# marzer/rt

Measured on AMD Instinct MI355X. Metric: Mrays/s (W*H*spp per second) and wall-clock, 1920x1080x256spp scenes/basic.toml, higher is better.
Workload: dtype f32

## Files before the change

rt_amd/csrc/kernels.hip:

```cpp
#include "kernels.hpp"
#include "contract.hpp"
#include "scan.hpp"
#include "bvh_scan.hpp"

#ifdef RT_HIP_FAST_BUILD
#define render_queue render_queue_fast
#define launch_render launch_render_fast
#endif

#include "../../include/rt_hip.h"

#include <algorithm>
#include <cstdlib>

#ifndef RT_HIP_WAVES_FEW
#define RT_HIP_WAVES_FEW 7
#endif
#ifndef RT_HIP_WAVES_MANY
#define RT_HIP_WAVES_MANY 6
#endif
#ifndef RT_HIP_WAVES_RESIDENT
#define RT_HIP_WAVES_RESIDENT 7
#endif
#ifndef RT_HIP_WAVES_DENSE
// ... 214 lines not shown
		}

		__device__ __forceinline__ uint32_t count_arrival(uint32_t* counter)
		{
#ifdef RT_HIP_MODEL_ORDERING
			return __hip_atomic_fetch_add(counter, 1u, __ATOMIC_RELEASE, __HIP_MEMORY_SCOPE_AGENT);
#else
			asm volatile("s_waitcnt vmcnt(0) ; what was published has left before the arrival is counted" ::: "memory");
			return __hip_atomic_fetch_add(counter, 1u, __ATOMIC_RELAXED, __HIP_MEMORY_SCOPE_AGENT);
#endif
		}
		__device__ __forceinline__ void last_arrival()
		{
#ifdef RT_HIP_MODEL_ORDERING
			__builtin_amdgcn_fence(__ATOMIC_ACQUIRE, "agent");
#else
			__builtin_amdgcn_fence(__ATOMIC_ACQUIRE, "wavefront");
#endif
		}

		template <int NS, bool SM, bool HALF = false, int NP = 0, bool GC = false>
		__global__ __launch_bounds__(block_threads, NS == -4 ? RT_HIP_WAVES_BVH : NS == -3 ? RT_HIP_WAVES_DENSE : (NS < 0 ? 5 : (NS == 0 ? RT_HIP_WAVES_RESIDENT : (NS >= 6 && NS + NP >= 7 ? RT_HIP_WAVES_MANY : RT_HIP_WAVES_FEW)))) void render_queue(const frame_params p,
																	  const queue_params q,
																	  const small_scene small,
																	  const device_scene s,
																	  const float4* __restrict__ geometry,
																	  uint32_t* __restrict__ out_rgba,
																	  float* __restrict__ out_rgb,
																	  device_counters* __restrict__ counters,
																	  unsigned long long* item_sums,
																	  uint32_t* pixel_done)
		{
			extern __shared__ float4 lds[];
			float4* const lds_geometry = lds;
			float4* const lds_shading = lds + scalar_max_spheres;
			constexpr bool RESIDENT = NS == 0;
			constexpr bool RESIDENT_SCALAR_SCAN = NS == 0 && NP == 1;
			const bool spheres_in_lds = RESIDENT && !RESIDENT_SCALAR_SCAN;
			const uint32_t lds_spheres = spheres_in_lds ? s.n_spheres : 0u;
			constexpr bool BVH = NS == -4;
			const uint32_t table_float4s = NS > 0 ? small_table_float4s : (RESIDENT ? lds_spheres + s.n_planes : (NS == -1 ? tile_primitives : (BVH ? bvh_stack_float4s : 0u)));
			if (NS > 0)
			{
				if (threadIdx.x == 0)
				{
#pragma unroll
					for (int i = 0; i < NS + NP; i++)
					{
						lds_geometry[i] = make_float4(small.geometry[i].x, small.geometry[i].y, small.geometry[i].z, __uint_as_float(small.scatter[i]));
						lds_shading[i] = small.shading[i];
					}
				}
			}
			else if (RESIDENT)
			{
				for (uint32_t i = threadIdx.x; i < lds_spheres + s.n_planes; i += block_threads)
					lds[i] = s.primitive_geometry[(s.n_spheres - lds_spheres) + i];
			}
			__syncthreads();

#ifdef RT_HIP_REGION_COUNTERS
			uint32_t region_runs[device_counters::regions] = {}, region_lanes[device_counters::regions] = {};
#endif
			constexpr bool ROLLING = NS < 0 && !BVH;
			device_bvh bvh{};
			if constexpr (BVH)
				bvh = *reinterpret_cast<const device_bvh*>(item_sums);
			constexpr bool RESIDENT_LDS_SCAN = NS == 0 && NP == 0;
			constexpr bool PINHOLE_ONLY = (NS > 0 || RESIDENT_LDS_SCAN) && !GC, EYE_ONLY = NS > 0 && GC, NEVER_PINHOLE = RESIDENT_LDS_SCAN && GC;
			const uint32_t lane = threadIdx.x & 63u;
			const uint32_t wave = threadIdx.x >> 6;
			const uint32_t chunk_items = q.chunks << q.pixels_log2;
			const uint32_t items = HALF ? 2u * chunk_items : chunk_items;
			constexpr uint32_t slot_floats = HALF ? half_chunk_slot_floats : 3u;
			float* const slots = reinterpret_cast<float*>(lds + table_float4s) + static_cast<size_t>(wave) * chunk_items * slot_floats;
			const uint32_t tile_w = 1u << q.tile_w_log2;
			const uint32_t tile_h = (1u << q.pixels_log2) >> q.tile_w_log2;

			const uint32_t tile_x0 = (blockIdx.x * 4u + wave) * tile_w;
			const uint32_t tile_y0 = (gridDim.y - 1u - blockIdx.y) * tile_h;
			uint32_t next_item = 0;

			const uint32_t items_per_pixel = (ROLLING && HALF) ? (p.samples_per_pixel + q.item_samples - 1u) / q.item_samples : q.chunks;
			const unsigned long long total_items = static_cast<unsigned long long>(p.width) * p.local_rows * items_per_pixel;
			unsigned long long block_next = 0, block_end = 0;
			unsigned long long prefetched = 0;
			uint32_t prefetched_count = ROLLING ? min(64u, q.lane_cap) : 64u;
			bool dry = false;
			if (ROLLING)
				prefetched = fetch_items(counters, prefetched_count);
#ifdef RT_HIP_WAVE_CLOCKS
			const unsigned long long clock_start = wall_clock64();
			unsigned long long clock_dry = 0;
#endif

			lane_state st;
			constexpr bool SCALAR_SEGMENTS = NS >= 1 && NS + NP <= 4;
			unsigned long long wave_segments = 0;
			uint32_t lane_segments = 0;
			uint32_t slot = 0;
			enum : uint32_t { lane_free = 0, lane_restart = 1, lane_retired = 3, lane_trace = 4 };
			uint32_t mode = lane_free;
#define RT_HIP_IS(m) ((m) == lane_trace ? mode >= lane_trace : mode == (m))
#define RT_HIP_BECOME(m) (mode = (m))

			const auto fold_tile = [&](const float* sums, uint32_t x0, uint32_t y0)
			{
				if (!ROLLING && (3u << q.pixels_log2) <= 64u)
				{
					const uint32_t channel = lane >> q.pixels_log2;
					const uint32_t pixel = lane & ((1u << q.pixels_log2) - 1u);
					const uint32_t lx = x0 + (pixel & (tile_w - 1u));
					const uint32_t ly = y0 + (pixel >> q.tile_w_log2);
					const bool live = channel < 3u && lx < p.width && ly < p.local_rows;
					float sum = 0.0f;
					if (live)
					{
						if (HALF)
						{
							for (uint32_t c = 0; c < q.chunks; c++)
							{
								const float* const slot_of_chunk = sums + ((c << q.pixels_log2) + pixel) * slot_floats;
								float chunk_sum = slot_of_chunk[channel];
								const uint32_t parked = parked_samples(p.samples_per_pixel, c);
								for (uint32_t j = 0; j < parked; j++)
									chunk_sum = chunk_sum + slot_of_chunk[3u + j * 3u + channel];
								sum = c ? sum + chunk_sum : chunk_sum;
							}
						}
						else
						{
							sum = sums[pixel * 3u + channel];
							for (uint32_t c = 1; c < q.chunks; c++)
								sum = sum + sums[((c << q.pixels_log2) + pixel) * 3u + channel];
						}
					}
					const float mean = sum / static_cast<float>(p.samples_per_pixel);
					const size_t o = static_cast<size_t>(output_row(live ? ly : 0u, p)) * p.width + lx;
					if (live && out_rgb)
						out_rgb[o * 3u + channel] = mean;
					const uint32_t byte = static_cast<uint32_t>(clamp01(__builtin_sqrtf(mean)) * 255.99999f);
					const uint32_t green = __shfl(byte, lane + (1u << q.pixels_log2), 64);
					const uint32_t blue = __shfl(byte, lane + (2u << q.pixels_log2), 64);
					if (live && channel == 0u)
						__hip_atomic_store(&out_rgba[o], (byte << 24u) | (green << 16u) | (blue << 8u) | 255u, __ATOMIC_RELAXED, __HIP_MEMORY_SCOPE_SYSTEM);
					return;
				}
				for (uint32_t pixel = lane; pixel < (1u << q.pixels_log2); pixel += 64u)
				{
					const uint32_t lx = x0 + (pixel & (tile_w - 1u));
					const uint32_t ly = y0 + (pixel >> q.tile_w_log2);
					if (lx < p.width && ly < p.local_rows)
					{
						vec3 colour = { 0.0f, 0.0f, 0.0f };
						if (HALF)
						{
							for (uint32_t c = 0; c < q.chunks; c++)
							{
								const float* const slot_of_chunk = sums + ((c << q.pixels_log2) + pixel) * slot_floats;
								vec3 chunk_sum = { slot_of_chunk[0], slot_of_chunk[1], slot_of_chunk[2] };
								const uint32_t parked = parked_samples(p.samples_per_pixel, c);
								for (uint32_t j = 0; j < parked; j++)
									chunk_sum = chunk_sum + vec3{ slot_of_chunk[3u + j * 3u], slot_of_chunk[4u + j * 3u], slot_of_chunk[5u + j * 3u] };
								colour = c ? colour + chunk_sum : chunk_sum;
							}
						}
						else
						{
							colour = { sums[pixel * 3u], sums[pixel * 3u + 1u], sums[pixel * 3u + 2u] };
							for (uint32_t c = 1; c < q.chunks; c++)
							{
								const uint32_t at = ((c << q.pixels_log2) + pixel) * 3u;
								colour = colour + vec3{ sums[at], sums[at + 1u], sums[at + 2u] };
							}
						}
						finish_pixel(colour, p, lx, ly, out_rgba, out_rgb);
					}
				}
			};
			const auto complete_item = [&]()
			{
				const uint32_t row = slot / p.width;
				const uint32_t lx = slot - row * p.width;
				const uint32_t ly = p.local_rows - 1u - row;
				if (HALF)
				{
					unsigned long long* const samples = item_sums + 2u * static_cast<size_t>(slot) * p.samples_per_pixel;
					const uint32_t before = count_arrival(&pixel_done[slot]);
					if (before + 1u == items_per_pixel)
					{
						last_arrival();
						vec3 colour = { 0.0f, 0.0f, 0.0f };
						for (uint32_t first = 0; first < p.samples_per_pixel; first += sample_chunk)
						{
							const uint32_t end = min(first + sample_chunk, p.samples_per_pixel);
							vec3 chunk_sum = { 0.0f, 0.0f, 0.0f };
							uint32_t i = first;
							for (; i + 8u <= end; i += 8u)
							{
								vec3 value[8];
								read_sums8(samples + 2u * i, value);
#pragma unroll
								for (uint32_t k = 0; k < 8u; k++)
									chunk_sum = chunk_sum + value[k];
							}
							for (; i < end; i++)
								chunk_sum = chunk_sum + read_sum(samples + 2u * i);
							colour = first ? colour + chunk_sum : chunk_sum;
						}
						finish_pixel(colour, p, lx, ly, out_rgba, out_rgb);
					}
					return;
				}
				if (q.chunks == 1u)
				{
					finish_pixel(st.chunk_sum, p, lx, ly, out_rgba, out_rgb);
					return;
				}
				const uint32_t chunk = (st.sample_end - 1u) / sample_chunk;
				unsigned long long* const sums = item_sums + 2u * static_cast<size_t>(slot) * q.chunks;
				publish_sum(sums + 2u * chunk, st.chunk_sum);
				const uint32_t before = count_arrival(&pixel_done[slot]);
				if (before + 1u == q.chunks)
				{
					last_arrival();
					vec3 colour = read_sum(sums);
					for (uint32_t c = 1; c < q.chunks; c++)
						colour = colour + read_sum(sums + 2u * c);
					finish_pixel(colour, p, lx, ly, out_rgba, out_rgb);
				}
			};

			constexpr bool INDEXED = HALF || ROLLING;
			const auto next_sample = [&]() -> bool
			{
#ifdef RT_HIP_FAST_BUILD
				st.window += st.keys.stride << draws_per_sample_log2;
#else
				asm("v_lshl_add_u32 %0, %1, %2, %0" : "+v"(st.window) : "v"(st.keys.stride), "n"(draws_per_sample_log2));
#endif
				if (INDEXED)
					return ++st.sample < st.sample_end;
				return st.window != st.window_end;
			};

			const auto end_sample = [&](vec3 contribution)
			{
				if (HALF && ROLLING)
				{
					publish_sum(item_sums + 2u * (static_cast<size_t>(slot) * p.samples_per_pixel + st.sample), contribution);
					if (next_sample())
						RT_HIP_BECOME(lane_restart);
					else
					{
						complete_item();
						RT_HIP_BECOME(lane_free);
					}
					return;
				}
				if (HALF)
				{
					const uint32_t half_chunk = slot >> q.pixels_log2;
					float* const slot_of_chunk = slots + ((((half_chunk >> 1u) << q.pixels_log2) + (slot & ((1u << q.pixels_log2) - 1u))) * slot_floats);
					if (st.sample & 8u)
					{
						float* const place = slot_of_chunk + 3u + (st.sample & 7u) * 3u;
						place[0] = contribution.x;
						place[1] = contribution.y;
						place[2] = contribution.z;
					}
					else
						st.chunk_sum = st.chunk_sum + contribution;
					if (next_sample())
						RT_HIP_BECOME(lane_restart);
					else
					{
						if (!((st.sample - 1u) & 8u))
						{
							slot_of_chunk[0] = st.chunk_sum.x;
							slot_of_chunk[1] = st.chunk_sum.y;
							slot_of_chunk[2] = st.chunk_sum.z;
						}
						RT_HIP_BECOME(lane_free);
					}
					return;
				}
				st.chunk_sum = st.chunk_sum + contribution;
				if (next_sample())
					RT_HIP_BECOME(lane_restart);
				else
				{
					if (ROLLING)
						complete_item();
					else
					{
						slots[slot * 3u + 0u] = st.chunk_sum.x;
						slots[slot * 3u + 1u] = st.chunk_sum.y;
						slots[slot * 3u + 2u] = st.chunk_sum.z;
					}
					RT_HIP_BECOME(lane_free);
				}
			};

			while (true)
			{
				RT_HIP_REGION(0);
				const bool tracing = RT_HIP_IS(lane_trace);
				if (SCALAR_SEGMENTS)
					wave_segments += static_cast<unsigned>(__builtin_popcountll(__builtin_amdgcn_ballot_w64(tracing)));
				candidate tiled_planes = { 0.0f, 0u, false };
				candidate tiled_spheres = { 0.0f, 0u, false };
				if (NS == -1 && __syncthreads_or(tracing))
				{
					for (uint32_t first = 0; first < s.n_planes; first += tile_primitives)
					{
						const uint32_t count = min(tile_primitives, s.n_planes - first);
						__syncthreads();
						stage_planes(lds, s, first, count);
						__syncthreads();
						if (tracing)
							scan_lds<false>(tiled_planes, st.origin, st.dir, lds, count, first);
					}
					for (uint32_t first = 0; first < s.n_spheres; first += tile_primitives)
					{
						const uint32_t count = min(tile_primitives, s.n_spheres - first);
						__syncthreads();
						stage_spheres(lds, s, first, count);
						__syncthreads();
						if (tracing)
							scan_lds<true>(tiled_spheres, st.origin, st.dir, lds, count, first);
					}
				}

				candidate together = { 0.0f, 0u, false };
				bool scanned_together = false;
#ifdef RT_HIP_NO_SPARSE_WAVES
				constexpr bool sparse_waves = false;
#else
				constexpr bool sparse_waves = true;
#endif
				if (sparse_waves && NS == -2 && s.n_spheres >= sparse_min_spheres)
				{
					unsigned long long holders = __builtin_amdgcn_ballot_w64(tracing);
					if (holders != 0 && static_cast<uint32_t>(__builtin_popcountll(holders)) <= q.sparse_rays)
					{
						while (holders != 0)
						{
							const int src = __builtin_ctzll(holders);
							holders &= holders - 1u;
							const vec3 o = { __int_as_float(__builtin_amdgcn_readlane(__float_as_int(st.origin.x), src)), __int_as_float(__builtin_amdgcn_readlane(__float_as_int(st.origin.y), src)),
											 __int_as_float(__builtin_amdgcn_readlane(__float_as_int(st.origin.z), src)) };
							const vec3 d = { __int_as_float(__builtin_amdgcn_readlane(__float_as_int(st.dir.x), src)), __int_as_float(__builtin_amdgcn_readlane(__float_as_int(st.dir.y), src)),
											 __int_as_float(__builtin_amdgcn_readlane(__float_as_int(st.dir.z), src)) };
							candidate found;
							const bool clean = scan_spheres_together(found, o, d, geometry, s.n_spheres, lane);
							if (clean && lane == static_cast<uint32_t>(src))
							{
								together = found;
								scanned_together = true;
							}
						}
					}
				}

				bool shade = false;
				vec3 normal;
				float4 shading;
				uint32_t scatter_kind = scatter_lambert;
				if (tracing)
				{
					RT_HIP_REGION(1);
					if (!SCALAR_SEGMENTS)
						lane_segments++;
					uint32_t kind;
					float distance;
					uint32_t small_index = 0;
					if (NS == -1)
					{
						uint32_t index;
						kind = select_hit(tiled_spheres, tiled_planes, distance, index);
						fetch_hit<SM>(s, st.origin, st.dir, kind, distance, index, normal, shading, scatter_kind);
					}
					else if (NS > 0)
					{
						candidate best = { 0.0f, 0u, false };
						constexpr int spheres_ns = NS > 0 ? NS : 1;
#ifdef RT_HIP_PROBE_GROUP
						constexpr int group = RT_HIP_PROBE_GROUP;
#else
						constexpr int group = spheres_ns <= 4 ? spheres_ns : 3;
#endif
#pragma unroll
						for (int first = 0; first < NS; first += group)
						{
							sphere_probe probes[group];
							unsigned long long lanes[group];
							unsigned long long any_lane = 0;
#pragma unroll
							for (int i = 0; i < group; i++)
								if (first + i < NS)
								{
									probes[i] = probe_sphere(st.origin, st.dir, small.geometry[first + i]);
									lanes[i] = __builtin_amdgcn_ballot_w64(probes[i].pos);
									any_lane |= lanes[i];
								}
							if (any_lane != 0)
							{
#pragma unroll
								for (int i = 0; i < group; i++)
									if (first + i < NS)
									{
										if (lanes[i] != 0)
											RT_HIP_REGION(2);
										finish_sphere(best, probes[i], small.geometry[first + i].w, static_cast<uint32_t>(first + i), lanes[i]);
									}
							}
						}
						if (NP > 0)
						{
							float plane_distance;
							uint32_t plane_slot = static_cast<uint32_t>(NS);
							bool plane;
							if (NP == 1)
								plane = test_one_plane(st.origin, st.dir, small.geometry[NS > 0 ? NS : 0], plane_distance);
							else
							{
								candidate best_plane = { 0.0f, 0u, false };
#pragma unroll
								for (int j = 0; j < NP; j++)
									test_plane(best_plane, st.origin, st.dir, small.geometry[(NS > 0 ? NS : 0) + j], static_cast<uint32_t>(j));
								plane = best_plane.have && best_plane.t >= 0.0f;
								plane_distance = best_plane.t;
								plane_slot += best_plane.index;
							}
							const bool nearer = best.t <= plane_distance;
							const bool sphere = best.have && best.t >= 0.0f;
							const bool use_sphere = sphere && (!plane || nearer);
							const bool use_plane = plane && !use_sphere;
							distance = use_sphere ? best.t : plane_distance;
							kind = use_sphere ? 1u : (use_plane ? 2u : 0u);
							small_index = use_sphere ? best.index : plane_slot;
						}
						else
						{
							const bool hit = best.have && best.t >= 0.0f;
							kind = hit ? 1u : 0u;
							distance = best.t;
							small_index = best.index;
						}
					}
					else
					{
						candidate planes = { 0.0f, 0u, false };
						candidate spheres = { 0.0f, 0u, false };
						const float4* const primitives = RESIDENT ? lds : geometry;
						scan_lds<false>(planes, st.origin, st.dir, RESIDENT ? lds + lds_spheres : geometry + s.n_spheres, s.n_planes, 0);
						if (BVH)
						{
							if (!bvh_spheres(spheres, st.origin, st.dir, bvh, geometry, reinterpret_cast<uint32_t*>(lds) + threadIdx.x))
							{
								spheres = { 0.0f, 0u, false };
								scan_streamed_spheres(spheres, st.origin, st.dir, geometry, s.n_spheres);
							}
#ifdef RT_HIP_BVH_CHECK
							candidate linear = { 0.0f, 0u, false };
							scan_streamed_spheres(linear, st.origin, st.dir, geometry, s.n_spheres);
							const bool same = linear.have == spheres.have && (!linear.have || (__float_as_uint(linear.t) == __float_as_uint(spheres.t) && linear.index == spheres.index));
							atomicAdd(&counters->bvh_checked, 1ull);
							if (!same)
								atomicAdd(&counters->bvh_disagreements, 1ull);
#endif
						}
						else if (NS == -2 || NS == -3)
						{
							if (scanned_together)
								spheres = together;
							else
								scan_streamed_spheres(spheres, st.origin, st.dir, geometry, s.n_spheres);
						}
						else if (RESIDENT_SCALAR_SCAN)
							scan_streamed_spheres(spheres, st.origin, st.dir, geometry, s.n_spheres);
						else
							scan_lds<true>(spheres, st.origin, st.dir, primitives, s.n_spheres, 0);
						uint32_t index;
						kind = select_hit(spheres, planes, distance, index);
						fetch_hit<SM>(s, st.origin, st.dir, kind, distance, index, normal, shading, scatter_kind);
					}
					if (!kind)
					{
						RT_HIP_REGION(4);
						end_sample(st.throughput * sky(st.dir.y));
					}
					else
					{
						shade = true;
						st.origin = ray_at(st.origin, st.dir, distance);
						if (NS > 0)
						{
							RT_HIP_REGION(3);
							const float4 g = lds_geometry[small_index];
							shading = lds_shading[small_index];
							scatter_kind = __float_as_uint(g.w);
							if (NP > 0 && kind == 2u)
								normal = { g.x, g.y, g.z };
							else
							{
								if (NP > 0)
									asm volatile("; hit: some lane hit a sphere" ::: "memory");
								normal = normalize(st.origin - vec3{ g.x, g.y, g.z });
							}
						}
					}
				}


				const unsigned long long asking = __builtin_amdgcn_ballot_w64(RT_HIP_IS(lane_free));
				const auto start_item = [&](uint32_t lx, uint32_t ly, uint32_t chunk)
				{
					const uint32_t item_samples = (HALF && ROLLING) ? q.item_samples : (HALF ? sample_chunk / 2u : sample_chunk);
					if (HALF && !ROLLING && chunk * item_samples >= p.samples_per_pixel)
						return;
					const uint32_t gy = global_row(ly, p);
					st.chunk_sum = { 0.0f, 0.0f, 0.0f };
					{
						const float fx = static_cast<float>(lx), fy = static_cast<float>(gy);
						if (PINHOLE_ONLY || (!EYE_ONLY && !NEVER_PINHOLE && p.pinhole))
						{
							st.base_x = fma(p.ray_d1[0], fx, fma(p.ray_d2[0], fy, p.ray_d0[0]));
							st.base_y = fma(p.ray_d1[1], fx, fma(p.ray_d2[1], fy, p.ray_d0[1]));
							st.base_z = fma(p.ray_d1[2], fx, fma(p.ray_d2[2], fy, p.ray_d0[2]));
							st.base_w = 0.0f;
						}
						else if (EYE_ONLY || p.eye_form)
						{
							st.base_x = fma(p.eye_q1[0], fx, fma(p.eye_q2[0], fy, p.eye_q0[0]));
							st.base_y = fma(p.eye_q1[1], fx, fma(p.eye_q2[1], fy, p.eye_q0[1]));
							st.base_z = fma(p.eye_q1[2], fx, fma(p.eye_q2[2], fy, p.eye_q0[2]));
							st.base_w = fma(p.eye_w1, fx, fma(p.eye_w2, fy, p.eye_w0));
						}
						else
						{
							st.base_x = fx, st.base_y = fy;
							st.base_z = st.base_w = 0.0f;
						}
					}
					st.keys.function_key = pixel_function_key(p.frame_key_a, gy * p.width + lx);
					st.keys.stride = pixel_stride(p.frame_key_b, st.keys.function_key);
					const uint32_t first = chunk * item_samples, end = min(first + item_samples, p.samples_per_pixel);
					st.sample = first;
					st.sample_end = end;
					st.window = sample_counter(st.keys.stride, first);
					st.window_end = sample_counter(st.keys.stride, end);
					RT_HIP_BECOME(lane_restart);
				};
				const auto take_item = [&](uint32_t item, uint32_t x0, uint32_t y0)
				{
					const uint32_t pixel = item & ((1u << q.pixels_log2) - 1u);
					const uint32_t chunk = item >> q.pixels_log2;
					const uint32_t lx = x0 + (pixel & (tile_w - 1u));
					const uint32_t ly = y0 + (pixel >> q.tile_w_log2);
					if (lx < p.width && ly < p.local_rows)
						start_item(lx, ly, chunk);
				};
				if (!ROLLING && asking != 0)
				{
					RT_HIP_REGION(6);
					const uint32_t rank = __builtin_amdgcn_mbcnt_hi(static_cast<uint32_t>(asking >> 32), __builtin_amdgcn_mbcnt_lo(static_cast<uint32_t>(asking), 0u));
					if (RT_HIP_IS(lane_free))
					{
						slot = next_item + rank;
						if (slot >= items)
							RT_HIP_BECOME(lane_retired);
						else
						{
							RT_HIP_REGION(7);
							take_item(slot, tile_x0, tile_y0);
						}
					}
					next_item += static_cast<uint32_t>(__builtin_popcountll(asking));
				}
				if (ROLLING && asking != 0)
				{
					const uint32_t rank = __builtin_amdgcn_mbcnt_hi(static_cast<uint32_t>(asking >> 32), __builtin_amdgcn_mbcnt_lo(static_cast<uint32_t>(asking), 0u));
					uint32_t want = static_cast<uint32_t>(__builtin_popcountll(asking));
					if (q.lane_cap < 64u)
					{
						const uint32_t holding = static_cast<uint32_t>(__builtin_popcountll(__builtin_amdgcn_ballot_w64(RT_HIP_IS(lane_trace) || RT_HIP_IS(lane_restart))));
						want = min(want, q.lane_cap > holding ? q.lane_cap - holding : 0u);
					}
					uint32_t served = 0;
					while (served < want)
					{
						if (block_next == block_end)
						{
							if (dry)
								break;
							if (prefetched >= total_items)
							{
								dry = true;
#ifdef RT_HIP_WAVE_CLOCKS
								clock_dry = wall_clock64();
#endif
								break;
							}
							block_next = prefetched;
							block_end = min(prefetched + prefetched_count, total_items);
// ... 687 lines not shown
```

rt_amd/csrc/scan.hpp:

```cpp
#pragma once

#include "contract.hpp"
#include "kernels.hpp"

namespace rt_hip
{
	constexpr uint32_t block_threads = 256;

	struct candidate
	{
		float t;
		uint32_t index;
		bool have;
	};

	struct sphere_probe
	{
		float a, e2, disc;
		bool pos;
	};

	__device__ __forceinline__ sphere_probe probe_sphere(vec3 o, vec3 d, float4 s)
	{
		const vec3 e = { s.x - o.x, s.y - o.y, s.z - o.z };
		sphere_probe p;
		p.a = dot(e, d);
		p.e2 = dot(e, e);
		p.disc = s.w - fma(-p.a, p.a, p.e2);
		p.pos = !(p.disc < 0.0f);
		return p;
	}

	__device__ __forceinline__ void finish_sphere(candidate& best, const sphere_probe& p, float r2, uint32_t index, unsigned long long lanes)
	{
		if (lanes != 0)
		{
			const float f = sqrt_rn_where(p.disc, p.pos);
			const float t = (p.e2 < r2) ? p.a + f : p.a - f;
			const bool accept = p.pos && !(t < min_hit_dist) && !(best.have && best.t <= t);
			best.t = accept ? t : best.t;
			best.index = accept ? index : best.index;
			best.have = best.have || accept;
		}
	}

	__device__ __forceinline__ void test_sphere(candidate& best, vec3 o, vec3 d, float4 s, uint32_t index)
	{
		const sphere_probe p = probe_sphere(o, d, s);
		finish_sphere(best, p, s.w, index, __builtin_amdgcn_ballot_w64(p.pos));
	}

	__device__ __forceinline__ void test_plane(candidate& best, vec3 o, vec3 d, float4 pl, uint32_t index)
	{
		const vec3 n = { pl.x, pl.y, pl.z };
		const float den = dot(n, d);
		const bool crosses = !(__builtin_fabsf(den) <= approx_zero_epsilon);
		const float num = dot(n, o) + pl.w;
		const float t = (-num) * rcp_rn_not_tiny_where(den, crosses);
		const bool accept = crosses && !(t < min_hit_dist) && !(best.have && best.t <= t);
		best.t = accept ? t : best.t;
		best.index = accept ? index : best.index;
		best.have = best.have || accept;
	}

	__device__ __forceinline__ bool test_one_plane(vec3 o, vec3 d, float4 pl, float& t)
	{
		const vec3 n = { pl.x, pl.y, pl.z };
		const float den = dot(n, d);
		const bool crosses = !(__builtin_fabsf(den) <= approx_zero_epsilon);
		const float num = dot(n, o) + pl.w;
		t = (-num) * rcp_in_band(den);
		return crosses && t >= min_hit_dist;
	}

	template <bool SPHERES>
	__device__ __forceinline__ void scan_lds(candidate& best, vec3 o, vec3 d, const float4* lds, uint32_t count, uint32_t first_index)
	{
		uint32_t i = 0;
		if (SPHERES)
		{
			for (; i + 4 <= count; i += 4)
			{
				const float4 s0 = lds[i], s1 = lds[i + 1], s2 = lds[i + 2], s3 = lds[i + 3];
				const sphere_probe p0 = probe_sphere(o, d, s0);
				const sphere_probe p1 = probe_sphere(o, d, s1);
				const sphere_probe p2 = probe_sphere(o, d, s2);
				const sphere_probe p3 = probe_sphere(o, d, s3);
				const unsigned long long m0 = __builtin_amdgcn_ballot_w64(p0.pos), m1 = __builtin_amdgcn_ballot_w64(p1.pos);
				const unsigned long long m2 = __builtin_amdgcn_ballot_w64(p2.pos), m3 = __builtin_amdgcn_ballot_w64(p3.pos);
				if ((m0 | m1 | m2 | m3) != 0)
				{
					finish_sphere(best, p0, s0.w, first_index + i, m0);
					finish_sphere(best, p1, s1.w, first_index + i + 1, m1);
					finish_sphere(best, p2, s2.w, first_index + i + 2, m2);
					finish_sphere(best, p3, s3.w, first_index + i + 3, m3);
				}
			}
		}
		for (; i < count; i++)
		{
			if (SPHERES)
				test_sphere(best, o, d, lds[i], first_index + i);
			else
				test_plane(best, o, d, lds[i], first_index + i);
		}
	}

	__device__ __forceinline__ void stage_spheres(float4* lds, const device_scene& s, uint32_t first, uint32_t count)
	{
		for (uint32_t i = threadIdx.x; i < count; i += block_threads)
		{
			const float r = s.sphere_r[first + i];
			lds[i] = make_float4(s.sphere_cx[first + i], s.sphere_cy[first + i], s.sphere_cz[first + i], r * r);
		}
	}

	__device__ __forceinline__ void stage_planes(float4* lds, const device_scene& s, uint32_t first, uint32_t count)
	{
		for (uint32_t i = threadIdx.x; i < count; i += block_threads)
			lds[i] = make_float4(s.plane_nx[first + i], s.plane_ny[first + i], s.plane_nz[first + i], s.plane_d[first + i]);
	}

	__device__ __forceinline__ uint32_t select_hit(const candidate& spheres, const candidate& planes, float& distance, uint32_t& index)
	{
		const float sphere_distance = spheres.have ? spheres.t : -1.0f;
		const float plane_distance = planes.have ? planes.t : -1.0f;
		const bool a = sphere_distance >= 0.0f;
		const bool b = plane_distance >= 0.0f;
		const bool use_sphere = a && (!b || sphere_distance <= plane_distance);
		const bool use_plane = !use_sphere && b;
		distance = use_sphere ? sphere_distance : (use_plane ? plane_distance : -1.0f);
		index = use_sphere ? spheres.index : planes.index;
		return use_sphere ? 1u : (use_plane ? 2u : 0u);
	}

	template <bool SM>
	__device__ __forceinline__ void
	fetch_hit(const device_scene& s, vec3 o, vec3 d, uint32_t kind, float distance, uint32_t index, vec3& normal, float4& shading, uint32_t& scatter)
	{
		scatter = scatter_lambert;
		if (kind)
		{
			const uint32_t primitive = kind == 1u ? index : s.n_spheres + index;
			const float4 g = s.primitive_geometry[primitive];
			shading = SM ? s.primitive_shading_sm[primitive] : s.primitive_shading[primitive];
			scatter = SM ? s.primitive_scatter_sm[primitive] : s.primitive_scatter[primitive];
			if (kind == 1u)
				normal = normalize(ray_at(o, d, distance) - vec3{ g.x, g.y, g.z });
			else
				normal = { g.x, g.y, g.z };
		}
	}
}
```

Before: 246,400.

## Add conservative sky-only tile test and fast sky-shading path for whole waves

Adds a conservative geometric test that checks whether a tile's pixel rectangle (padded for jitter) can only see sky, against every sphere and plane of a small scene. When every lane in a wave agrees the tile sees only sky, the wave skips the full trace state machine and directly accumulates sky colour for each sample using the same RNG-derived jitter, then writes chunk sums to slots. This removes intersection and bounce work for sky-only tiles, at the cost of extra per-tile test arithmetic and more code and registers in the kernel. Correctness depends on the conservative margins bounding every ray in the tile.

New measurement: 240,400. 0.976x the previous value.

```diff
diff --git a/rt_amd/csrc/kernels.hip b/rt_amd/csrc/kernels.hip
--- a/rt_amd/csrc/kernels.hip
+++ b/rt_amd/csrc/kernels.hip
@@ -540,6 +540,78 @@
 				}
 			};
 
+#ifdef RT_HIP_NO_SKY_WAVES
+			constexpr bool SKY_WAVES = false;
+#else
+			constexpr bool SKY_WAVES = NS > 0 && PINHOLE_ONLY && !HALF;
+#endif
+			bool sky_wave = false;
+			if constexpr (SKY_WAVES)
+			{
+				const float y_lo = static_cast<float>(global_row(tile_y0, p)), y_hi = static_cast<float>(global_row(tile_y0 + tile_h - 1u, p) + 1u);
+				const bool only_sky = q.pixels_log2 <= 6u && rectangle_sees_only_sky<(NS > 0 ? NS : 0), NP>(p, small, static_cast<float>(tile_x0), static_cast<float>(tile_x0 + tile_w), y_lo, y_hi);
+				sky_wave = __builtin_amdgcn_ballot_w64(!only_sky) == 0;
+			}
+			if (sky_wave)
+			{
+				const uint32_t pixel = lane & ((1u << q.pixels_log2) - 1u);
+				const uint32_t lx = tile_x0 + (pixel & (tile_w - 1u));
+				const uint32_t ly = tile_y0 + (pixel >> q.tile_w_log2);
+				if (lx < p.width && ly < p.local_rows)
+				{
+					const uint32_t gy = global_row(ly, p);
+					const float fx = static_cast<float>(lx), fy = static_cast<float>(gy);
+					const vec3 base = { fma(p.ray_d1[0], fx, fma(p.ray_d2[0], fy, p.ray_d0[0])), fma(p.ray_d1[1], fx, fma(p.ray_d2[1], fy, p.ray_d0[1])),
+										fma(p.ray_d1[2], fx, fma(p.ray_d2[2], fy, p.ray_d0[2])) };
+					stream_keys keys;
+					keys.function_key = pixel_function_key(p.frame_key_a, gy * p.width + lx);
+					keys.stride = pixel_stride(p.frame_key_b, keys.function_key);
+					for (uint32_t chunk = lane >> q.pixels_log2; chunk < q.chunks; chunk += 64u >> q.pixels_log2)
+					{
+						const uint32_t first = chunk * sample_chunk, end = min(first + sample_chunk, p.samples_per_pixel);
+						uint32_t window = sample_counter(keys.stride, first);
+						const uint32_t window_end = sample_counter(keys.stride, end);
+						vec3 chunk_sum = { 0.0f, 0.0f, 0.0f };
+						do
+						{
+							const uint32_t word = step_word_at(window + keys.stride, keys);
+							float jx = step_numerator(word * step_mul_a), jy = step_numerator(word * step_mul_b);
+							if (__builtin_amdgcn_ballot_w64(window == 0u) != 0)
+							{
+								asm volatile("; sky: some lane is at its pixel's sample 0" ::: "memory");
+								if (window == 0u)
+									jx = jy = 0x1.0p23f;
+							}
+							const vec3 toward = { fma(p.ray_j1[0], jx, fma(p.ray_j2[0], jy, base.x)), fma(p.ray_j1[1], jx, fma(p.ray_j2[1], jy, base.y)),
+												  fma(p.ray_j1[2], jx, fma(p.ray_j2[2], jy, base.z)) };
+							float dir_y = toward.y * inv_sqrt_rn(dot(toward, toward));
+#ifdef RT_HIP_FAST_BUILD
+							asm volatile("" : "+v"(dir_y));
+#endif
+							chunk_sum = chunk_sum + sky(dir_y);
+							window += keys.stride << draws_per_sample_log2;
+						}
+						while (window != window_end);
+						const uint32_t item = (chunk << q.pixels_log2) + pixel;
+						slots[item * 3u + 0u] = chunk_sum.x;
+						slots[item * 3u + 1u] = chunk_sum.y;
+						slots[item * 3u + 2u] = chunk_sum.z;
+					}
+				}
+				const uint32_t columns = tile_x0 < p.width ? min(tile_w, p.width - tile_x0) : 0u;
+				const uint32_t rows = tile_y0 < p.local_rows ? min(tile_h, p.local_rows - tile_y0) : 0u;
+				const uint32_t traced = columns * rows * p.samples_per_pixel;
+#ifdef RT_HIP_COUNT_SKY_WAVES
+				const uint32_t reported = traced + columns * rows;
+#else
+				const uint32_t reported = traced;
+#endif
+				if (SCALAR_SEGMENTS)
+					wave_segments = reported;
+				else
+					lane_segments = lane == 0u ? reported : 0u;
+			}
+			else
 			while (true)
 			{
 				RT_HIP_REGION(0);
diff --git a/rt_amd/csrc/scan.hpp b/rt_amd/csrc/scan.hpp
--- a/rt_amd/csrc/scan.hpp
+++ b/rt_amd/csrc/scan.hpp
@@ -121,6 +121,66 @@
 			lds[i] = make_float4(s.plane_nx[first + i], s.plane_ny[first + i], s.plane_nz[first + i], s.plane_d[first + i]);
 	}
 
+	constexpr float sky_jitter_pad = 0.0625f;
+	constexpr float sky_margin = 0x1.0p-15f;
+
+	template <int NS, int NP>
+	__device__ __forceinline__ bool rectangle_sees_only_sky(const frame_params& p, const small_scene& small, float x_lo, float x_hi, float y_lo, float y_hi)
+	{
+		const float cx = 0.5f * (x_lo + x_hi), cy = 0.5f * (y_lo + y_hi);
+		const float hx = fma(0.5f, x_hi - x_lo, sky_jitter_pad), hy = fma(0.5f, y_hi - y_lo, sky_jitter_pad);
+		const vec3 d1 = { p.ray_d1[0], p.ray_d1[1], p.ray_d1[2] }, d2 = { p.ray_d2[0], p.ray_d2[1], p.ray_d2[2] };
+		const vec3 eye = { p.ray_eye[0], p.ray_eye[1], p.ray_eye[2] };
+		const vec3 c = { fma(d1.x, cx, fma(d2.x, cy, p.ray_d0[0])), fma(d1.y, cx, fma(d2.y, cy, p.ray_d0[1])), fma(d1.z, cx, fma(d2.z, cy, p.ray_d0[2])) };
+		const float rho2 = fma(hx * hx, dot(d1, d1), fma(hy * hy, dot(d2, d2), (2.0f * hx * hy) * __builtin_fabsf(dot(d1, d2))));
+		const float rho = sqrt_rn(rho2) * 1.001f;
+		const float c2 = dot(c, c), cd1 = dot(c, d1), cd2 = dot(c, d2);
+		const float c_len = sqrt_rn(c2);
+		const float t_max = c_len + rho, t_min = c_len - rho;
+		const float t_max2 = t_max * t_max, t_min2 = t_min * t_min;
+		const float eye1 = __builtin_fabsf(eye.x) + __builtin_fabsf(eye.y) + __builtin_fabsf(eye.z);
+		bool sky = t_min > 0.0f && t_max2 < 0x1.0p60f;
+#pragma unroll
+		for (int i = 0; i < NS; i++)
+		{
+			const float4 s = small.geometry[i];
+			const vec3 e = { s.x - eye.x, s.y - eye.y, s.z - eye.z };
+			const float e2 = dot(e, e), ec = dot(e, c);
+			const float e_len = sqrt_rn(e2);
+			const float m0 = (__builtin_fabsf(s.x) + __builtin_fabsf(s.y) + __builtin_fabsf(s.z)) + (eye1 + t_max);
+			const float scale2 = fma(m0, m0, s.w);
+			const float pad2 = sky_margin * scale2;
+			const float r2p = s.w + pad2;
+			const float k = e2 - r2p;
+			const float ed1 = dot(e, d1), ed2 = dot(e, d2);
+			const float spread = fma(hx, __builtin_fabsf(ed1), hy * __builtin_fabsf(ed2)) * 1.001f;
+			const float reach = spread + __builtin_fabsf(ec);
+			const float ahead = spread + ec;
+			const float outside = e_len - t_max;
+			const float x2 = fma(e2, c2, -(ec * ec));
+			const float sway = fma(hx, __builtin_fabsf(fma(e2, cd1, -(ec * ed1))), hy * __builtin_fabsf(fma(e2, cd2, -(ec * ed2)))) * 1.001f;
+			const float clear = x2 - sway;
+			const bool line = k * t_min2 > reach * reach || (clear > 0.0f && clear * clear > (r2p * t_max2) * x2);
+			const bool behind = ahead < 0.0f && ahead * ahead > (sky_margin * pad2) * t_max2 && outside > 0.0f && outside * outside > r2p;
+			sky = sky && e2 + scale2 < 0x1.0p60f && k > 0.0f && (line || behind);
+		}
+#pragma unroll
+		for (int j = 0; j < NP; j++)
+		{
+			const float4 pl = small.geometry[NS + j];
+			const vec3 n = { pl.x, pl.y, pl.z };
+			const float n1 = __builtin_fabsf(n.x) + __builtin_fabsf(n.y) + __builtin_fabsf(n.z);
+			const float s0 = dot(n, eye) + pl.w, nc = dot(n, c);
+			const float spread = n1 * rho;
+			const float room_s = sky_margin * fma(n1, eye1 + t_max, __builtin_fabsf(pl.w));
+			const float room_d = sky_margin * (n1 * t_max);
+			const bool above = s0 > room_s && nc - spread > room_d;
+			const bool below = -s0 > room_s && -(nc + spread) > room_d;
+			sky = sky && n1 + __builtin_fabsf(pl.w) + eye1 < 0x1.0p60f && (above || below);
+		}
+		return sky;
+	}
+
 	__device__ __forceinline__ uint32_t select_hit(const candidate& spheres, const candidate& planes, float& distance, uint32_t& index)
 	{
 		const float sphere_distance = spheres.have ? spheres.t : -1.0f;
```
